# mmorel-35/trivy

Measured on AMD Instinct MI355X. Metric: GB/s secret-scanned (builtin rules) at 1/2/4/8 MI355X; findings diff = 0, higher is better.
Workload: dtype u8

## Files before the change

trivy_amd/csrc/capi.cpp:

```cpp
#include "../../include/trivy_secret.h"
#include "../../include/trivy_secret_test.h"

#include <algorithm>
#include <atomic>
#include <chrono>
#include <memory>
#include <cstdio>
#include <cstdlib>
#include <cstring>
#include <deque>
#include <condition_variable>
#include <mutex>
#include <thread>

#include <malloc.h>
#include <pthread.h>

#include "engine.h"
#include "gosort.h"
#include "guard.h"
#include "inflate_dev.h"
#include "feed.h"
#include "tar.h"
#include "tarscan.h"
// ... 939 lines not shown
  in.paths = paths;
  in.path_lens = path_lens;
  in.binary = binary;
  std::unique_ptr<tsg_result> r(new tsg_result());
  r->rs = rs->rs;
  RawScan raw;
  const std::function<void()> before_confirm = [&] { if (release) release(user); };
  if (!eng->model_scan_device(in, chunk, &r->files, &r->stats, &err, &raw, &before_confirm))
    return fail(TSG_ERR_INTERNAL, err);
  r->raw_segs = std::move(raw.segs);
  *out = r.release();
  return TSG_OK;
  TSG_API_CATCH
}

int tsg_result_raw_segments(const tsg_result* r, size_t* n) {
  TSG_API_TRY
  if (!r || !n) return fail(TSG_ERR_INVALID, "NULL argument");
  *n = r->raw_segs.size();
  return TSG_OK;
  TSG_API_CATCH
}

int tsg_result_raw_segment(const tsg_result* r, size_t k, tsg_raw_segment* rec) {
  TSG_API_TRY
  if (!r || !rec) return fail(TSG_ERR_INVALID, "NULL argument");
  if (k >= r->raw_segs.size()) return fail(TSG_ERR_INVALID, "no such segment");
  const RawSegment& s = r->raw_segs[k];
  rec->f0 = s.f0; rec->nfiles = s.nfiles; rec->lead = s.lead; rec->chunk_bytes = s.chunk;
  rec->b0 = s.b0; rec->bytes = s.bytes; rec->lead_bytes = s.lead_bytes; rec->hits = s.hits;
  rec->lead_flags = s.lead_flags; rec->lead_emitted = s.lead_emitted;
  rec->chunk_newlines = s.nl.data(); rec->nchunks = s.nl.size();
  rec->lead_cand_rules = s.lead_rules.data(); rec->lead_cand_starts = s.lead_starts.data();
  rec->nlead_cands = s.lead_rules.size();
  return TSG_OK;
  TSG_API_CATCH
}

int tsg_test_inject_segment_failures(tsg_engine* e, uint32_t n) {
  TSG_API_TRY
  if (!e) return fail(TSG_ERR_INVALID, "engine is NULL");
  e->eng->inject_segment_failures(n);
  return TSG_OK;
  TSG_API_CATCH
}

int tsg_test_wire_pack(const uint8_t* src, size_t n, int path, uint8_t* packed, size_t packed_cap, uint32_t* table,
                       size_t* packed_len, int* path_used, uint8_t* back) {
  TSG_API_TRY
  if ((!src && n) || !table || !packed_len || (!packed && packed_cap)) return fail(TSG_ERR_INVALID, "NULL argument");
  if (path < 0 || path > 2 || n > kWireMaxStrip) return fail(TSG_ERR_INVALID, "path or length out of range");
  std::vector<uint8_t> buf(wire_bound(n));
  std::vector<uint32_t> tab(wire_blocks(n) + 1);
  const size_t pl = wire_pack(src, n, buf.data(), tab.data(), path);
  *packed_len = pl;
  if (path_used) *path_used = path != kWireScalar && wire_have_avx2() ? kWireAvx2 : kWireScalar;
  if (pl > packed_cap) return fail(TSG_ERR_INVALID, "packed_cap is too small");
  if (pl) memcpy(packed, buf.data(), pl);
  memcpy(table, tab.data(), wire_blocks(n) * sizeof(uint32_t));
  if (back) {
    std::vector<uint8_t> exact(buf.begin(), buf.begin() + pl);
    wire_unpack(exact.data(), tab.data(), n, back);
  }
  return TSG_OK;
  TSG_API_CATCH
}

int tsg_test_wire_unpack_device(const uint8_t* packed, size_t packed_len, const uint32_t* table, size_t n,
                                uint8_t* out) {
  TSG_API_TRY
  if (n && (!packed || !table || !out)) return fail(TSG_ERR_INVALID, "NULL argument");
  const char* msg = "";
  if (!wire_unpack_device_probe(packed, packed_len, table, n, out, &msg)) return fail(TSG_ERR_INTERNAL, msg);
  return TSG_OK;
  TSG_API_CATCH
}

static int test_wire_pack2(const uint8_t* src, size_t n, int path, bool split, uint8_t* packed, size_t packed_cap,
                           uint32_t* table, uint8_t* alpha, size_t* packed_len, int* path_used, uint64_t* counts,
                           uint8_t* back) {
  TSG_API_TRY
  if ((!src && n) || !table || !alpha || !packed_len || (!packed && packed_cap)) return fail(TSG_ERR_INVALID, "NULL argument");
  if (path < 0 || path > 3 || n > kWireMaxStrip) return fail(TSG_ERR_INVALID, "path or length out of range");
  std::vector<uint8_t> buf(wire2_bound(n));
  std::vector<uint32_t> tab(wire_blocks(n) + 1);
  std::vector<uint8_t> al(wire2_alpha_bytes(n) + 1);
  Wire2Stats st;
  const size_t pl = wire_pack2(src, n, buf.data(), tab.data(), al.data(), path, &st, split);
  *packed_len = pl;
  if (path_used) *path_used = wire2_path(path);
  if (counts) { counts[0] = st.blocks6; counts[1] = st.blocks7; counts[2] = st.blocks_raw; counts[3] = st.escaped; }
  if (counts && split) counts[4] = st.blocks_split;
  if (pl > packed_cap) return fail(TSG_ERR_INVALID, "packed_cap is too small");
  if (pl) memcpy(packed, buf.data(), pl);
  memcpy(table, tab.data(), wire_blocks(n) * sizeof(uint32_t));
  memcpy(alpha, al.data(), wire2_alpha_bytes(n));
  if (back) {
    std::vector<uint8_t> exact(buf.begin(), buf.begin() + pl);
    wire_unpack2(exact.data(), tab.data(), al.data(), n, back);
  }
  return TSG_OK;
  TSG_API_CATCH
}

int tsg_test_wire_pack2(const uint8_t* src, size_t n, int path, uint8_t* packed, size_t packed_cap, uint32_t* table,
                        uint8_t* alpha, size_t* packed_len, int* path_used, uint64_t* counts, uint8_t* back) {
  return test_wire_pack2(src, n, path, false, packed, packed_cap, table, alpha, packed_len, path_used, counts, back);
}

int tsg_test_wire_pack3(const uint8_t* src, size_t n, int path, uint8_t* packed, size_t packed_cap, uint32_t* table,
                        uint8_t* alpha, size_t* packed_len, int* path_used, int* vbmi2, uint64_t* counts, uint8_t* back) {
  if (vbmi2) *vbmi2 = wire_have_vbmi2() ? 1 : 0;
  return test_wire_pack2(src, n, path, true, packed, packed_cap, table, alpha, packed_len, path_used, counts, back);
}

int tsg_test_wire_unpack2_device(const uint8_t* packed, size_t packed_len, const uint32_t* table, const uint8_t* alpha,
                                 size_t n, uint8_t* out) {
  TSG_API_TRY
  if (n && (!packed || !table || !alpha || !out)) return fail(TSG_ERR_INVALID, "NULL argument");
  const char* msg = "";
  if (!wire_unpack2_device_probe(packed, packed_len, table, alpha, n, out, &msg)) return fail(TSG_ERR_INTERNAL, msg);
  return TSG_OK;
  TSG_API_CATCH
}

int tsg_test_wire_unpack3_device(const uint8_t* packed, size_t packed_len, const uint32_t* table, const uint8_t* alpha,
                                 size_t n, uint8_t* out) {
  return tsg_test_wire_unpack2_device(packed, packed_len, table, alpha, n, out);
}

static std::string cstr(const char* p) { return p ? std::string(p) : std::string(); }

int tsg_result_from_json(const char* json, size_t len, tsg_result** out) {
  TSG_API_TRY
  if (!json || !out) return fail(TSG_ERR_INVALID, "NULL argument");
  JValue doc;
  std::string err;
  if (!json_parse(std::string(json, len), &doc, &err) || doc.kind != JValue::Arr) return fail(TSG_ERR_INVALID, "json: " + err);
  auto* r = new tsg_result();
  r->own_rules = std::make_shared<std::deque<Rule>>();
  auto sget = [](const JValue* o, const char* k) { const JValue* v = o ? o->get(k) : nullptr; return v ? v->as_string() : std::string(); };
  auto iget = [](const JValue* o, const char* k) { const JValue* v = o ? o->get(k) : nullptr; return v && v->kind == JValue::Num ? static_cast<int>(v->num) : 0; };
  auto bget = [](const JValue* o, const char* k) { const JValue* v = o ? o->get(k) : nullptr; return v && v->kind == JValue::Bool && v->b; };
  auto put = [](SecretBuilder* s, const std::string& v) { return s->put(v.data(), v.size()); };
  for (const auto& js : doc.arr) {
    SecretBuilder s;
    s.file_path = sget(&js, "FilePath");
    const JValue* fs = js.get("Findings");
    if (fs && fs->kind == JValue::Arr) {
      for (const auto& jf : fs->arr) {
        Rule rule;
        rule.id = sget(&jf, "RuleID");
        rule.category = sget(&jf, "Category");
        rule.title = sget(&jf, "Title");
        rule.severity = sget(&jf, "Severity");
        r->own_rules->push_back(rule);
        FindingRec f;
        f.rule = &r->own_rules->back();
        f.start_line = iget(&jf, "StartLine");
        f.end_line = iget(&jf, "EndLine");
        f.match = put(&s, sget(&jf, "Match"));
        f.line_begin = static_cast<uint32_t>(s.lines.size());
        const JValue* code = jf.get("Code");
        const JValue* lines = code ? code->get("Lines") : nullptr;
        if (lines && lines->kind == JValue::Arr) {
          for (const auto& jl : lines->arr) {
            LineRec ln;
            ln.number = iget(&jl, "Number");
            ln.content = put(&s, sget(&jl, "Content"));
            ln.is_cause = bget(&jl, "IsCause");
            ln.first_cause = bget(&jl, "FirstCause");
            ln.last_cause = bget(&jl, "LastCause");
// ... 984 lines not shown
```

trivy_amd/csrc/wirepack.cpp:

```cpp
#include "wirepack.h"

#include <algorithm>
#include <cstring>
#include <memory>

#if defined(__x86_64__)
#include <immintrin.h>
#endif

namespace tsg {

namespace {

constexpr uint64_t kHigh = 0x8080808080808080ull;

inline uint64_t squeeze(uint64_t x) {
  x = (x & 0x007F007F007F007Full) | ((x & 0x7F007F007F007F00ull) >> 1);
  x = (x & 0x00003FFF00003FFFull) | ((x & 0x3FFF00003FFF0000ull) >> 2);
  return (x & 0x000000000FFFFFFFull) | ((x & 0x0FFFFFFF00000000ull) >> 4);
}

inline uint64_t spread(uint64_t v) {
  uint64_t x = (v & 0x000000000FFFFFFFull) | ((v << 4) & 0x0FFFFFFF00000000ull);
  x = (x & 0x00003FFF00003FFFull) | ((x << 2) & 0x3FFF00003FFF0000ull);
  return (x & 0x007F007F007F007Full) | ((x << 1) & 0x7F007F007F007F00ull);
}

inline uint64_t pack_groups_scalar(const uint8_t* src, size_t n, size_t g0, uint8_t* dst) {
  uint64_t acc = 0;
  const size_t ng = n / 8;
  for (size_t g = g0; g < ng; ++g) {
    uint64_t x;
    std::memcpy(&x, src + 8 * g, 8);
    acc |= x;
    x = squeeze(x & ~kHigh);
    std::memcpy(dst + 7 * g, &x, 8);
  }
  if (n % 8) {
    uint64_t x = 0;
    std::memcpy(&x, src + 8 * ng, n % 8);
    acc |= x;
    x = squeeze(x & ~kHigh);
    std::memcpy(dst + 7 * ng, &x, 8);
  }
  return acc;
}

uint64_t pack_block_scalar(const uint8_t* src, size_t n, uint8_t* dst) { return pack_groups_scalar(src, n, 0, dst); }

#if defined(__x86_64__)
__attribute__((target("avx2"))) uint64_t pack_block_avx2(const uint8_t* src, size_t n, uint8_t* dst) {
  const __m256i m1 = _mm256_set1_epi64x(0x007F007F007F007Fll), m1h = _mm256_set1_epi64x(0x7F007F007F007F00ll);
  const __m256i m2 = _mm256_set1_epi64x(0x00003FFF00003FFFll), m2h = _mm256_set1_epi64x(0x3FFF00003FFF0000ll);
  const __m256i m3 = _mm256_set1_epi64x(0x000000000FFFFFFFll), m3h = _mm256_set1_epi64x(0x0FFFFFFF00000000ll);
  const __m256i shuf = _mm256_setr_epi8(0, 1, 2, 3, 4, 5, 6, 8, 9, 10, 11, 12, 13, 14, -1, -1,
                                        0, 1, 2, 3, 4, 5, 6, 8, 9, 10, 11, 12, 13, 14, -1, -1);
  __m256i acc = _mm256_setzero_si256();
  const size_t nv = n / 32;
  for (size_t i = 0; i < nv; ++i) {
    __m256i x = _mm256_loadu_si256(reinterpret_cast<const __m256i*>(src + 32 * i));
    acc = _mm256_or_si256(acc, x);
    x = _mm256_or_si256(_mm256_and_si256(x, m1), _mm256_srli_epi64(_mm256_and_si256(x, m1h), 1));
    x = _mm256_or_si256(_mm256_and_si256(x, m2), _mm256_srli_epi64(_mm256_and_si256(x, m2h), 2));
    x = _mm256_or_si256(_mm256_and_si256(x, m3), _mm256_srli_epi64(_mm256_and_si256(x, m3h), 4));
    x = _mm256_shuffle_epi8(x, shuf);
    _mm_storeu_si128(reinterpret_cast<__m128i*>(dst + 28 * i), _mm256_castsi256_si128(x));
    _mm_storeu_si128(reinterpret_cast<__m128i*>(dst + 28 * i + 14), _mm256_extracti128_si256(x, 1));
  }
  const __m128i a = _mm_or_si128(_mm256_castsi256_si128(acc), _mm256_extracti128_si256(acc, 1));
  uint64_t r = static_cast<uint64_t>(_mm_cvtsi128_si64(a)) | static_cast<uint64_t>(_mm_extract_epi64(a, 1));
  return r | pack_groups_scalar(src, n, nv * 4, dst);
}
#endif

}

bool wire_have_avx2() {
#if defined(__x86_64__)
  static const bool have = __builtin_cpu_supports("avx2");
  return have;
#else
  return false;
#endif
}

size_t wire_pack(const uint8_t* src, size_t n, uint8_t* dst, uint32_t* table, int path) {
  uint64_t (*pack_block)(const uint8_t*, size_t, uint8_t*) = pack_block_scalar;
#if defined(__x86_64__)
  if (path != kWireScalar && wire_have_avx2()) pack_block = pack_block_avx2;
#endif
  size_t o = 0;
  const size_t nb = wire_blocks(n);
  for (size_t b = 0; b < nb; ++b) {
    const uint8_t* s = src + b * kWireBlock;
    const size_t len = n - b * kWireBlock < kWireBlock ? n - b * kWireBlock : kWireBlock;
    if (pack_block(s, len, dst + o) & kHigh) {
      std::memcpy(dst + o, s, len);
      table[b] = static_cast<uint32_t>(o) | kWireRawBit;
      o += len;
    } else {
      table[b] = static_cast<uint32_t>(o);
      o += wire_packed_len(len);
    }
  }
  return o;
}

namespace {

void unpack7_block(const uint8_t* s, size_t len, uint8_t* d) {
  for (size_t g = 0; 8 * g < len; ++g) {
    uint64_t v = 0;
    std::memcpy(&v, s + 7 * g, 7);
    const uint64_t x = spread(v);
    std::memcpy(d + 8 * g, &x, len - 8 * g < 8 ? len - 8 * g : 8);
  }
}

}

void wire_unpack(const uint8_t* packed, const uint32_t* table, size_t n, uint8_t* dst) {
  const size_t nb = wire_blocks(n);
  for (size_t b = 0; b < nb; ++b) {
    const size_t len = n - b * kWireBlock < kWireBlock ? n - b * kWireBlock : kWireBlock;
    const uint8_t* s = packed + (table[b] & ~kWireRawBit);
    uint8_t* d = dst + b * kWireBlock;
    if (table[b] & kWireRawBit) {
      std::memcpy(d, s, len);
      continue;
    }
    unpack7_block(s, len, d);
  }
}


namespace {

constexpr uint32_t kAbort = ~0u;

struct Alphabet {
  uint8_t code[256];
  alignas(64) uint8_t inv[128];
};

void choose_alphabet(const uint8_t* p, size_t len, uint8_t* vals, Alphabet* a) {
  uint32_t key[128];
  for (uint32_t v = 0; v < 128; ++v) key[v] = 127 - v;
  for (size_t i = 0; i < len; i += kWire2Sample)
    if (p[i] < 0x80) key[p[i]] += 256;
  std::partial_sort(key, key + kWire2Escape, key + 128, [](uint32_t x, uint32_t y) { return x > y; });
  std::memset(a->code, kWire2Escape, sizeof a->code);
  std::memset(a->inv, 0, sizeof a->inv);
  for (uint32_t c = 0; c < kWire2Escape; ++c) {
    const uint8_t v = static_cast<uint8_t>(127 - (key[c] & 0xFF));
    vals[c] = v;
    a->code[v] = static_cast<uint8_t>(c);
    a->inv[v] = static_cast<uint8_t>(kWire2Escape - c);
  }
  vals[kWire2Escape] = 0;
}

inline uint32_t pack6_groups_scalar(const uint8_t* src, size_t len, size_t g0, const Alphabet& a, uint8_t* dst,
                                    uint8_t* esc, uint32_t nesc, uint32_t limit, uint32_t* acc) {
  const size_t ng = (len + 3) / 4;
  for (size_t g = g0; g < ng; ++g) {
    uint32_t v = 0;
    const size_t k = len - 4 * g < 4 ? len - 4 * g : 4;
    for (size_t j = 0; j < k; ++j) {
      const uint8_t x = src[4 * g + j];
      const uint32_t c = a.code[x];
      *acc |= x;
      v |= c << (6 * j);
      if (c == kWire2Escape) esc[nesc++] = x;
    }
    dst[3 * g] = static_cast<uint8_t>(v);
    dst[3 * g + 1] = static_cast<uint8_t>(v >> 8);
    dst[3 * g + 2] = static_cast<uint8_t>(v >> 16);
    if (nesc >= limit) return kAbort;
  }
  return nesc;
}

uint32_t pack6_scalar(const uint8_t* src, size_t len, const Alphabet& a, uint8_t* dst, uint8_t* esc, uint32_t limit,
                      uint32_t* acc) {
  return pack6_groups_scalar(src, len, 0, a, dst, esc, 0, limit, acc);
}

#if defined(__x86_64__)
__attribute__((target("avx2"))) uint32_t pack6_avx2(const uint8_t* src, size_t len, const Alphabet& a, uint8_t* dst,
                                                     uint8_t* esc, uint32_t limit, uint32_t* acc) {
  __m256i T[8], X[8];
  for (int k = 0; k < 8; ++k) {
    T[k] = _mm256_broadcastsi128_si256(_mm_load_si128(reinterpret_cast<const __m128i*>(a.inv + 16 * k)));
    X[k] = _mm256_set1_epi8(static_cast<char>(16 * k));
  }
  const __m256i k70 = _mm256_set1_epi8(0x70), k63 = _mm256_set1_epi8(63);
  const __m256i mul1 = _mm256_set1_epi16(0x4001), mul2 = _mm256_set1_epi32(0x10000001);
  const __m256i shuf = _mm256_setr_epi8(0, 1, 2, 4, 5, 6, 8, 9, 10, 12, 13, 14, -1, -1, -1, -1,
                                        0, 1, 2, 4, 5, 6, 8, 9, 10, 12, 13, 14, -1, -1, -1, -1);
  __m256i vacc = _mm256_setzero_si256();
  uint32_t nesc = 0;
  const size_t nv = len / 32;
  for (size_t i = 0; i < nv; ++i) {
    const __m256i x = _mm256_loadu_si256(reinterpret_cast<const __m256i*>(src + 32 * i));
    vacc = _mm256_or_si256(vacc, x);
    __m256i r = _mm256_shuffle_epi8(T[0], _mm256_adds_epu8(x, k70));
    for (int k = 1; k < 8; ++k)
      r = _mm256_or_si256(r, _mm256_shuffle_epi8(T[k], _mm256_adds_epu8(_mm256_xor_si256(x, X[k]), k70)));
    const __m256i c = _mm256_sub_epi8(k63, r);
    uint32_t m = static_cast<uint32_t>(_mm256_movemask_epi8(_mm256_cmpeq_epi8(c, k63)));
    __m256i p = _mm256_madd_epi16(_mm256_maddubs_epi16(c, mul1), mul2);
    p = _mm256_shuffle_epi8(p, shuf);
    _mm_storeu_si128(reinterpret_cast<__m128i*>(dst + 24 * i), _mm256_castsi256_si128(p));
    _mm_storeu_si128(reinterpret_cast<__m128i*>(dst + 24 * i + 12), _mm256_extracti128_si256(p, 1));
    if (m) {
      for (; m; m &= m - 1) esc[nesc++] = src[32 * i + static_cast<unsigned>(__builtin_ctz(m))];
      if (nesc >= limit) return kAbort;
    }
  }
  const __m128i v = _mm_or_si128(_mm256_castsi256_si128(vacc), _mm256_extracti128_si256(vacc, 1));
  const uint64_t r = static_cast<uint64_t>(_mm_cvtsi128_si64(v)) | static_cast<uint64_t>(_mm_extract_epi64(v, 1));
  *acc |= (r & kHigh) ? 0x80u : 0u;
  return pack6_groups_scalar(src, len, nv * 8, a, dst, esc, nesc, limit, acc);
}

__attribute__((target("avx512f,avx512bw,avx512vl,avx512vbmi"))) uint32_t pack6_vbmi(const uint8_t* src, size_t len,
                                                                                     const Alphabet& a, uint8_t* dst,
                                                                                     uint8_t* esc, uint32_t limit,
                                                                                     uint32_t* acc) {
  const __m512i t0 = _mm512_load_si512(a.inv), t1 = _mm512_load_si512(a.inv + 64);
  const __m512i k63 = _mm512_set1_epi8(63);
  const __m512i mul1 = _mm512_set1_epi16(0x4001), mul2 = _mm512_set1_epi32(0x10000001);
  alignas(64) uint8_t idx[64];
  for (int j = 0; j < 64; ++j) idx[j] = static_cast<uint8_t>(j < 48 ? j / 3 * 4 + j % 3 : 0);
  const __m512i gather = _mm512_load_si512(idx);
  __mmask64 high = 0;
  uint32_t nesc = 0;
  const size_t nv = len / 64;
  for (size_t i = 0; i < nv; ++i) {
// ... 48 lines not shown
#endif


struct Split {
  alignas(64) uint8_t mask[kWireBlock / 8 + 64];
  alignas(64) uint8_t nib[kWireBlock + 128];
  alignas(64) uint8_t five[kWireBlock + 128];
  alignas(64) uint8_t esc[kWireBlock + 128];
  uint32_t h = 0, e = 0;
  uint32_t e6 = 0;
  bool high = false;
};

inline void split_finish(Split* s, size_t len, uint32_t h, uint32_t e, uint32_t e6, bool high) {
  std::memset(s->nib + h, 0, 64);
  std::memset(s->five + (len - h), 0, 64);
  s->h = h; s->e = e; s->e6 = e6; s->high = high;
}

inline void split_scan_codes(const uint8_t* src, const uint8_t* code, size_t i0, size_t len, Split* s, uint32_t h,
                             uint32_t e, uint32_t e6, uint32_t acc) {
  uint32_t w = static_cast<uint32_t>(i0) - h;
  for (size_t i = i0; i < len; ++i) {
    const uint8_t x = src[i], c = code[i];
    acc |= x;
    if (i % 8 == 0) s->mask[i / 8] = 0;
    if (c < kWire2Hot) {
      s->mask[i / 8] |= static_cast<uint8_t>(1u << (i % 8));
      s->nib[h++] = c;
    } else if (c < kWire2Warm) {
      s->five[w++] = static_cast<uint8_t>(c - kWire2Hot);
    } else {
      s->five[w++] = kWire2Escape5;
      s->esc[e++] = x;
      e6 += c == kWire2Escape;
    }
  }
  split_finish(s, len, h, e, e6, (acc & 0x80) != 0);
}

void split_scan_scalar(const uint8_t* src, size_t len, const Alphabet& a, Split* s) {
  uint8_t code[kWireBlock];
  for (size_t i = 0; i < len; ++i) code[i] = a.code[src[i]];
  split_scan_codes(src, code, 0, len, s, 0, 0, 0, 0);
}

void split_emit_scalar(const Split& s, size_t len, uint8_t* d) {
  const size_t M = (len + 7) / 8, N = (s.h + 1) / 2, nf = len - s.h, F = (5 * nf + 7) / 8;
  std::memcpy(d, s.mask, M);
  d += M;
  for (size_t j = 0; j < N; ++j) d[j] = static_cast<uint8_t>(s.nib[2 * j] | s.nib[2 * j + 1] << 4);
  d += N;
  for (size_t g = 0; 5 * g < F; ++g) {
    uint64_t v = 0;
    for (int j = 0; j < 8; ++j) v |= static_cast<uint64_t>(s.five[8 * g + j]) << (5 * j);
    for (size_t j = 0; j < 5 && 5 * g + j < F; ++j) d[5 * g + j] = static_cast<uint8_t>(v >> (8 * j));
  }
  d += F;
  std::memcpy(d, s.esc, s.e);
  std::memset(d + s.e, 0, wire2_split_bytes(len, s.h, s.e) - (M + N + F + s.e));
}

#if defined(__x86_64__)
__attribute__((target("avx2"))) void split_scan_avx2(const uint8_t* src, size_t len, const Alphabet& a, Split* s) {
  __m256i T[8], X[8];
  for (int k = 0; k < 8; ++k) {
    T[k] = _mm256_broadcastsi128_si256(_mm_load_si128(reinterpret_cast<const __m128i*>(a.inv + 16 * k)));
    X[k] = _mm256_set1_epi8(static_cast<char>(16 * k));
  }
  const __m256i k70 = _mm256_set1_epi8(0x70), k63 = _mm256_set1_epi8(63);
  alignas(32) uint8_t code[kWireBlock];
  const size_t nv = len / 32;
  for (size_t i = 0; i < nv; ++i) {
    const __m256i x = _mm256_loadu_si256(reinterpret_cast<const __m256i*>(src + 32 * i));
    __m256i r = _mm256_shuffle_epi8(T[0], _mm256_adds_epu8(x, k70));
    for (int k = 1; k < 8; ++k)
      r = _mm256_or_si256(r, _mm256_shuffle_epi8(T[k], _mm256_adds_epu8(_mm256_xor_si256(x, X[k]), k70)));
    _mm256_store_si256(reinterpret_cast<__m256i*>(code + 32 * i), _mm256_sub_epi8(k63, r));
  }
  for (size_t i = 32 * nv; i < len; ++i) code[i] = a.code[src[i]];
  split_scan_codes(src, code, 0, len, s, 0, 0, 0, 0);
}

__attribute__((target("avx512f,avx512bw,avx512vl,avx512vbmi,avx512vbmi2"))) void split_scan_vbmi2(
    const uint8_t* src, size_t len, const Alphabet& a, Split* s) {
  const __m512i t0 = _mm512_load_si512(a.inv), t1 = _mm512_load_si512(a.inv + 64);
  const __m512i k63 = _mm512_set1_epi8(63), khot = _mm512_set1_epi8(static_cast<char>(kWire2Hot));
  const __m512i kwarm = _mm512_set1_epi8(static_cast<char>(kWire2Warm)), k31 = _mm512_set1_epi8(kWire2Escape5);
  uint32_t h = 0, w = 0, e = 0, e6 = 0;
  __mmask64 high = 0;
  for (size_t i = 0; i < len; i += 64) {
    const __mmask64 valid = len - i >= 64 ? ~0ull : (1ull << (len - i)) - 1;
    const __m512i x = _mm512_maskz_loadu_epi8(valid, src + i);
    const __mmask64 hi = _mm512_movepi8_mask(x);
    high |= hi;
    const __m512i r = _mm512_permutex2var_epi8(t0, x, t1);
    const __m512i c = _mm512_mask_mov_epi8(_mm512_sub_epi8(k63, r), hi, k63);
    const __mmask64 hot = _mm512_cmplt_epu8_mask(c, khot) & valid, rest = ~hot & valid;
    const uint64_t hot_bits = hot;
    std::memcpy(s->mask + i / 8, &hot_bits, 8);
    _mm512_storeu_si512(s->nib + h, _mm512_maskz_compress_epi8(hot, c));
    h += static_cast<uint32_t>(__builtin_popcountll(hot));
    const __m512i f = _mm512_min_epu8(_mm512_sub_epi8(c, khot), k31);
    _mm512_storeu_si512(s->five + w, _mm512_maskz_compress_epi8(rest, f));
    w += static_cast<uint32_t>(__builtin_popcountll(rest));
    const __mmask64 out = _mm512_cmpge_epu8_mask(c, kwarm) & valid;
    if (out) {
      _mm512_storeu_si512(s->esc + e, _mm512_maskz_compress_epi8(out, x));
      e += static_cast<uint32_t>(__builtin_popcountll(out));
      e6 += static_cast<uint32_t>(__builtin_popcountll(_mm512_cmpeq_epi8_mask(c, k63) & valid));
    }
  }
  split_finish(s, len, h, e, e6, high != 0);
}

__attribute__((target("avx512f,avx512bw,avx512vl,avx512vbmi"))) void split_emit_vbmi(const Split& s, size_t len,
                                                                                     uint8_t* d) {
  const size_t M = (len + 7) / 8, N = (s.h + 1) / 2, nf = len - s.h, F = (5 * nf + 7) / 8;
  std::memcpy(d, s.mask, M);
  d += M;
  const __m512i two = _mm512_set1_epi16(0x1001);
  for (size_t j = 0; j < s.h; j += 64) {
    const __m512i v = _mm512_load_si512(s.nib + j);
    _mm256_storeu_si256(reinterpret_cast<__m256i*>(d + j / 2), _mm512_cvtepi16_epi8(_mm512_maddubs_epi16(v, two)));
  }
  d += N;
  alignas(64) uint8_t idx[64];
  for (int j = 0; j < 64; ++j) idx[j] = static_cast<uint8_t>(j < 40 ? j / 5 * 8 + j % 5 : 5);
  const __m512i gather = _mm512_load_si512(idx);
  const __m512i mul1 = _mm512_set1_epi16(0x2001), mul2 = _mm512_set1_epi32(0x04000001);
  const __m512i lo20 = _mm512_set1_epi64(0xFFFFF), hi20 = _mm512_set1_epi64(0xFFFFF00000ll);
  for (size_t j = 0; j < nf; j += 64) {
    const __m512i v = _mm512_load_si512(s.five + j);
    const __m512i q = _mm512_madd_epi16(_mm512_maddubs_epi16(v, mul1), mul2);
    const __m512i p = _mm512_or_si512(_mm512_and_si512(q, lo20), _mm512_and_si512(_mm512_srli_epi64(q, 12), hi20));
    _mm512_storeu_si512(d + j / 8 * 5, _mm512_permutexvar_epi8(gather, p));
  }
  d += F;
  std::memcpy(d, s.esc, s.e);
  std::memset(d + s.e, 0, wire2_split_bytes(len, s.h, s.e) - (M + N + F + s.e));
}
#endif

}

bool wire_have_vbmi() {
#if defined(__x86_64__)
  static const bool have = __builtin_cpu_supports("avx512f") && __builtin_cpu_supports("avx512bw") &&
                           __builtin_cpu_supports("avx512vl") && __builtin_cpu_supports("avx512vbmi");
  return have;
#else
  return false;
#endif
}

bool wire_have_vbmi2() {
#if defined(__x86_64__)
  static const bool have = wire_have_vbmi() && __builtin_cpu_supports("avx512vbmi2");
  return have;
#else
  return false;
#endif
}

int wire2_path(int path) {
  if (path == kWireScalar) return kWireScalar;
  if (path != kWireAvx2 && wire_have_vbmi()) return kWireVbmi;
  return wire_have_avx2() ? kWireAvx2 : kWireScalar;
}

size_t wire_pack2(const uint8_t* src, size_t n, uint8_t* dst, uint32_t* table, uint8_t* alpha, int path,
                  Wire2Stats* stats, bool split) {
  uint32_t (*pack6)(const uint8_t*, size_t, const Alphabet&, uint8_t*, uint8_t*, uint32_t, uint32_t*) = pack6_scalar;
  uint64_t (*pack7)(const uint8_t*, size_t, uint8_t*) = pack_block_scalar;
  void (*split_scan)(const uint8_t*, size_t, const Alphabet&, Split*) = split_scan_scalar;
  void (*split_emit)(const Split&, size_t, uint8_t*) = split_emit_scalar;
#if defined(__x86_64__)
  const int used = wire2_path(path);
  if (used != kWireScalar) pack7 = pack_block_avx2;
  if (used == kWireAvx2) pack6 = pack6_avx2;
  if (used == kWireVbmi) pack6 = wire_have_vbmi2() ? pack6_vbmi2 : pack6_vbmi;
  if (used != kWireScalar) { split_scan = split_scan_avx2; }
  if (used == kWireVbmi) split_emit = split_emit_vbmi;
  if (used == kWireVbmi && wire_have_vbmi2()) split_scan = split_scan_vbmi2;
#endif
  if (n) std::memset(alpha, 0, wire2_alpha_bytes(n));
  Wire2Stats st;
  Alphabet a;
  uint8_t esc[kWireBlock + 64];
  std::unique_ptr<Split> sp(split ? new Split : nullptr);
  size_t o = 0;
  const size_t nb = wire_blocks(n);
  for (size_t b = 0; b < nb; ++b) {
    const size_t at = b * kWireBlock;
    if (at % kWire2Region == 0)
      choose_alphabet(src + at, n - at < kWire2Region ? n - at : kWire2Region, alpha + at / kWire2Region * kWire2Alpha, &a);
    const uint8_t* s = src + at;
    const size_t len = n - at < kWireBlock ? n - at : kWireBlock;
    const size_t cb = wire2_code_bytes(len);
    const uint32_t limit = len > cb ? static_cast<uint32_t>(len - cb) : 0;
    uint32_t acc = 0;
    bool no6 = false;
    if (split) {
      split_scan(s, len, a, sp.get());
      const size_t size7 = sp->high ? len : wire_packed_len(len), size6 = cb + ((sp->e6 + 15) & ~size_t(15));
      const size_t sizes = wire2_split_bytes(len, sp->h, sp->e);
      if (sizes < len && sizes < size7 && sizes < size6) {
        split_emit(*sp, len, dst + o);
        table[b] = static_cast<uint32_t>(o) | kWireRawBit | kWire6Bit;
        o += sizes;
        ++st.blocks_split;
        st.escaped += sp->e;
        continue;
      }
      no6 = !(size6 < len && size6 < size7);
    }
    const uint32_t nesc = limit && !no6 ? pack6(s, len, a, dst + o, esc, limit, &acc) : kAbort;
    if (nesc != kAbort) {
      const size_t size6 = cb + ((nesc + 15) & ~size_t(15));
      const bool ascii = !(acc & 0x80);
      if (size6 < len && !(ascii && wire_packed_len(len) <= size6)) {
        const size_t codes = (len + 3) / 4 * 3;
        std::memset(dst + o + codes, 0, cb - codes);
        std::memcpy(dst + o + cb, esc, nesc);
        std::memset(dst + o + cb + nesc, 0, size6 - cb - nesc);
        table[b] = static_cast<uint32_t>(o) | kWire6Bit;
        o += size6;
        ++st.blocks6;
        st.escaped += nesc;
        continue;
      }
    }
    if (wire_packed_len(len) < len && !(pack7(s, len, dst + o) & kHigh)) {
      table[b] = static_cast<uint32_t>(o);
      o += wire_packed_len(len);
      ++st.blocks7;
    } else {
      std::memcpy(dst + o, s, len);
      table[b] = static_cast<uint32_t>(o) | kWireRawBit;
      o += len;
      ++st.blocks_raw;
    }
  }
  if (stats) *stats = st;
  return o;
}

void wire_unpack2(const uint8_t* packed, const uint32_t* table, const uint8_t* alpha, size_t n, uint8_t* dst) {
  const size_t nb = wire_blocks(n);
  for (size_t b = 0; b < nb; ++b) {
    const size_t at = b * kWireBlock;
    const size_t len = n - at < kWireBlock ? n - at : kWireBlock;
    const uint8_t* s = packed + (table[b] & ~(kWireRawBit | kWire6Bit));
    uint8_t* d = dst + at;
    if ((table[b] & kWireRawBit) && (table[b] & kWire6Bit)) {
      const uint8_t* al = alpha + at / kWire2Region * kWire2Alpha;
      size_t h = 0;
      for (size_t i = 0; i < len; ++i) h += s[i / 8] >> (i % 8) & 1;
      const uint8_t* nib = s + (len + 7) / 8;
      const uint8_t* five = nib + (h + 1) / 2;
      const uint8_t* e = five + (5 * (len - h) + 7) / 8;
      size_t jn = 0, jf = 0;
      for (size_t i = 0; i < len; ++i) {
        if (s[i / 8] >> (i % 8) & 1) {
          d[i] = al[nib[jn / 2] >> (4 * (jn % 2)) & 15];
          ++jn;
        } else {
          const size_t bit = 5 * jf++;
          const uint32_t lo = five[bit >> 3], hi = (bit & 7) > 3 ? five[(bit >> 3) + 1] : 0;
          const uint32_t c = ((lo | hi << 8) >> (bit & 7)) & 31;
          d[i] = c == kWire2Escape5 ? *e++ : al[kWire2Hot + c];
        }
      }
    } else if (table[b] & kWireRawBit) {
      std::memcpy(d, s, len);
    } else if (table[b] & kWire6Bit) {
      const uint8_t* al = alpha + at / kWire2Region * kWire2Alpha;
      const uint8_t* e = s + wire2_code_bytes(len);
      for (size_t i = 0; i < len; ++i) {
        const size_t bit = 6 * i;
        const uint32_t lo = s[bit >> 3], hi = (bit & 7) > 2 ? s[(bit >> 3) + 1] : 0;
        const uint32_t c = ((lo | hi << 8) >> (bit & 7)) & 63;
        d[i] = c == kWire2Escape ? *e++ : al[c];
      }
    } else {
      unpack7_block(s, len, d);
    }
  }
}

}
```

trivy_amd/csrc/wirepack.h:

```cpp
#pragma once
#include <cstddef>
#include <cstdint>

namespace tsg {

constexpr uint32_t kWireBlock = 4096;
constexpr uint32_t kWireBlockPacked = kWireBlock / 8 * 7;
constexpr uint32_t kWireRawBit = 1u << 31;
constexpr uint64_t kWireMaxStrip = 1ull << 30;
constexpr size_t kWireSlack = 64;

enum WirePath { kWireAuto = 0, kWireScalar = 1, kWireAvx2 = 2, kWireVbmi = 3 };

inline size_t wire_blocks(size_t n) { return (n + kWireBlock - 1) / kWireBlock; }
inline size_t wire_packed_len(size_t block_bytes) { return (block_bytes + 7) / 8 * 7; }
inline size_t wire_bound(size_t n) { return n + 8 + kWireSlack; }
inline size_t wire_table_bytes(size_t n) { return (wire_blocks(n) * sizeof(uint32_t) + 255) & ~size_t(255); }

bool wire_have_avx2();
size_t wire_pack(const uint8_t* src, size_t n, uint8_t* dst, uint32_t* table, int path);
void wire_unpack(const uint8_t* packed, const uint32_t* table, size_t n, uint8_t* dst);

bool wire_unpack_device_probe(const uint8_t* packed, size_t packed_len, const uint32_t* table, size_t n, uint8_t* out,
                              const char** err);


constexpr uint32_t kWire6Bit = 1u << 30;
constexpr uint32_t kWire2Region = 65536;
constexpr uint32_t kWire2Sample = 64;
constexpr uint32_t kWire2Alpha = 64;
constexpr uint32_t kWire2Escape = 63;

struct Wire2Stats {
  uint64_t blocks6 = 0, blocks7 = 0, blocks_raw = 0;
  uint64_t escaped = 0;
  uint64_t blocks_split = 0;
};

inline size_t wire2_regions(size_t n) { return (n + kWire2Region - 1) / kWire2Region; }
inline size_t wire2_alpha_bytes(size_t n) { return (wire2_regions(n) * kWire2Alpha + 255) & ~size_t(255); }
inline size_t wire2_code_bytes(size_t block_bytes) { return ((block_bytes + 3) / 4 * 3 + 15) & ~size_t(15); }
inline size_t wire2_bound(size_t n) { return n + 16 + kWireSlack; }
constexpr uint32_t kWire2Hot = 16;
constexpr uint32_t kWire2Warm = 47;
constexpr uint32_t kWire2Escape5 = 31;
inline size_t wire2_split_bytes(size_t len, size_t h, size_t e) {
  return ((len + 7) / 8 + (h + 1) / 2 + (5 * (len - h) + 7) / 8 + e + 15) & ~size_t(15);
}

bool wire_have_vbmi();
bool wire_have_vbmi2();
int wire2_path(int path);
size_t wire_pack2(const uint8_t* src, size_t n, uint8_t* dst, uint32_t* table, uint8_t* alpha, int path,
                  Wire2Stats* stats, bool split = false);
void wire_unpack2(const uint8_t* packed, const uint32_t* table, const uint8_t* alpha, size_t n, uint8_t* dst);
bool wire_unpack2_device_probe(const uint8_t* packed, size_t packed_len, const uint32_t* table, const uint8_t* alpha,
                               size_t n, uint8_t* out, const char** err);

}
```

Before: 74.28.

## Vectorize wire2 split scan/emit with AVX-512 and speed up alphabet ranking

Replaces the split-mode host packing path with AVX-512 VBMI2 routines: a scan that stores codes, nibble and 5-bit values plus escapes into a new VScan buffer, then vectorized nibble/five-bit packing and a 6-bit code emitter. It also adds an optional merge variant that packs on the fly, a histogram-plus-SIMD ranking in place of partial_sort for alphabet choice, and software prefetch of upcoming source and destination. The intent is to cut host-side CPU cost of wire compression before device upload. It adds complexity and scratch memory, and ordering ties in the rank path could differ from partial_sort.

```diff
diff --git a/trivy_amd/csrc/capi.cpp b/trivy_amd/csrc/capi.cpp
--- a/trivy_amd/csrc/capi.cpp
+++ b/trivy_amd/csrc/capi.cpp
@@ -1045,12 +1045,15 @@
   TSG_API_TRY
   if ((!src && n) || !table || !alpha || !packed_len || (!packed && packed_cap)) return fail(TSG_ERR_INVALID, "NULL argument");
   if (path < 0 || path > 3 || n > kWireMaxStrip) return fail(TSG_ERR_INVALID, "path or length out of range");
-  std::vector<uint8_t> buf(wire2_bound(n));
+  constexpr size_t kGuard = 64;
+  std::vector<uint8_t> buf(wire2_bound(n) + kGuard, 0xA5);
   std::vector<uint32_t> tab(wire_blocks(n) + 1);
   std::vector<uint8_t> al(wire2_alpha_bytes(n) + 1);
   Wire2Stats st;
   const size_t pl = wire_pack2(src, n, buf.data(), tab.data(), al.data(), path, &st, split);
   *packed_len = pl;
+  for (size_t i = 0; i < kGuard; ++i)
+    if (buf[wire2_bound(n) + i] != 0xA5) return fail(TSG_ERR_INTERNAL, "wire_pack2 wrote past wire2_bound(n)");
   if (path_used) *path_used = wire2_path(path);
   if (counts) { counts[0] = st.blocks6; counts[1] = st.blocks7; counts[2] = st.blocks_raw; counts[3] = st.escaped; }
   if (counts && split) counts[4] = st.blocks_split;
diff --git a/trivy_amd/csrc/wirepack.cpp b/trivy_amd/csrc/wirepack.cpp
--- a/trivy_amd/csrc/wirepack.cpp
+++ b/trivy_amd/csrc/wirepack.cpp
@@ -2,6 +2,7 @@
 
 #include <algorithm>
 #include <cstring>
+#include <functional>
 #include <memory>
 
 #if defined(__x86_64__)
@@ -137,24 +138,71 @@
 namespace {
 
 constexpr uint32_t kAbort = ~0u;
+#ifndef TSG_WIRE_PREFETCH
+#define TSG_WIRE_PREFETCH 1
+#endif
+constexpr bool kWirePrefetch = TSG_WIRE_PREFETCH != 0;
 
 struct Alphabet {
   uint8_t code[256];
   alignas(64) uint8_t inv[128];
 };
 
-void choose_alphabet(const uint8_t* p, size_t len, uint8_t* vals, Alphabet* a) {
-  uint32_t key[128];
-  for (uint32_t v = 0; v < 128; ++v) key[v] = 127 - v;
-  for (size_t i = 0; i < len; i += kWire2Sample)
-    if (p[i] < 0x80) key[p[i]] += 256;
-  std::partial_sort(key, key + kWire2Escape, key + 128, [](uint32_t x, uint32_t y) { return x > y; });
-  std::memset(a->code, kWire2Escape, sizeof a->code);
+#if defined(__x86_64__)
+__attribute__((target("avx512f,avx512bw,avx512vl"))) void rank_keys_avx512(const uint32_t* key, uint8_t* rank) {
+  __m512i K[8], R[8];
+  for (int j = 0; j < 8; ++j) {
+    K[j] = _mm512_load_si512(key + 16 * j);
+    R[j] = _mm512_setzero_si512();
+  }
+  const __m512i one = _mm512_set1_epi32(1);
+  for (int v = 0; v < 128; ++v) {
+    const __m512i b = _mm512_set1_epi32(static_cast<int>(key[v]));
+    for (int j = 0; j < 8; ++j) R[j] = _mm512_mask_add_epi32(R[j], _mm512_cmpgt_epu32_mask(b, K[j]), R[j], one);
+  }
+  for (int j = 0; j < 8; ++j) _mm_store_si128(reinterpret_cast<__m128i*>(rank + 16 * j), _mm512_cvtepi32_epi8(R[j]));
+}
+#endif
+
+void choose_alphabet(const uint8_t* p, size_t len, uint8_t* vals, Alphabet* a, bool want_code) {
+  uint16_t hist[4][128];
+  std::memset(hist, 0, sizeof hist);
+  const size_t ns = (len + kWire2Sample - 1) / kWire2Sample;
+  size_t s = 0;
+  for (; s + 4 <= ns; s += 4) {
+    const uint8_t b0 = p[kWire2Sample * s], b1 = p[kWire2Sample * (s + 1)];
+    const uint8_t b2 = p[kWire2Sample * (s + 2)], b3 = p[kWire2Sample * (s + 3)];
+    hist[0][b0 & 127] += static_cast<uint16_t>((b0 >> 7) ^ 1);
+    hist[1][b1 & 127] += static_cast<uint16_t>((b1 >> 7) ^ 1);
+    hist[2][b2 & 127] += static_cast<uint16_t>((b2 >> 7) ^ 1);
+    hist[3][b3 & 127] += static_cast<uint16_t>((b3 >> 7) ^ 1);
+  }
+  for (; s < ns; ++s) hist[0][p[kWire2Sample * s] & 127] += static_cast<uint16_t>((p[kWire2Sample * s] >> 7) ^ 1);
+  alignas(64) uint32_t key[128];
+  for (uint32_t v = 0; v < 128; ++v)
+    key[v] = static_cast<uint32_t>(hist[0][v] + hist[1][v] + hist[2][v] + hist[3][v]) << 8 | (127 - v);
+  if (want_code) std::memset(a->code, kWire2Escape, sizeof a->code);
   std::memset(a->inv, 0, sizeof a->inv);
+#if defined(__x86_64__)
+  if (wire_have_vbmi()) {
+    alignas(64) uint8_t rank[128], order[128];
+    rank_keys_avx512(key, rank);
+    for (uint32_t v = 0; v < 128; ++v) {
+      const uint32_t c = rank[v];
+      order[c] = static_cast<uint8_t>(v);
+      a->inv[v] = static_cast<uint8_t>(c < kWire2Escape ? kWire2Escape - c : 0);
+      if (want_code) a->code[v] = static_cast<uint8_t>(c < kWire2Escape ? c : kWire2Escape);
+    }
+    std::memcpy(vals, order, kWire2Escape);
+    vals[kWire2Escape] = 0;
+    return;
+  }
+#endif
+  std::partial_sort(key, key + kWire2Escape, key + 128, std::greater<uint32_t>());
   for (uint32_t c = 0; c < kWire2Escape; ++c) {
     const uint8_t v = static_cast<uint8_t>(127 - (key[c] & 0xFF));
     vals[c] = v;
-    a->code[v] = static_cast<uint8_t>(c);
+    if (want_code) a->code[v] = static_cast<uint8_t>(c);
     a->inv[v] = static_cast<uint8_t>(kWire2Escape - c);
   }
   vals[kWire2Escape] = 0;
@@ -369,36 +417,177 @@
   split_scan_codes(src, code, 0, len, s, 0, 0, 0, 0);
 }
 
-__attribute__((target("avx512f,avx512bw,avx512vl,avx512vbmi,avx512vbmi2"))) void split_scan_vbmi2(
-    const uint8_t* src, size_t len, const Alphabet& a, Split* s) {
+struct VScan {
+  alignas(64) uint8_t esc[kWireBlock + 64];
+  alignas(64) uint8_t code[kWireBlock];
+  alignas(64) uint8_t nib[kWireBlock + 128];
+  alignas(64) uint8_t val5[kWireBlock + 128];
+  alignas(64) uint8_t five[kWireBlock / 8 * 5 + 64];
+  uint32_t h = 0, e = 0, e6 = 0;
+  bool high = false;
+};
+
+struct VTables {
+  alignas(64) uint8_t rotate[64][64];
+  alignas(64) uint64_t waiting[128];
+  alignas(64) uint8_t gather4[64], gather5[64], gather6[64];
+  constexpr VTables() : rotate(), waiting(), gather4(), gather5(), gather6() {
+    for (int w = 0; w < 64; ++w) {
+      for (int j = 0; j < 64; ++j) rotate[w][j] = static_cast<uint8_t>((j - w) & 63);
+      waiting[w] = (1ull << w) - 1;
+    }
+    for (int j = 0; j < 64; ++j) {
+      gather4[j] = static_cast<uint8_t>(j < 32 ? 2 * j : 1);
+      gather5[j] = static_cast<uint8_t>(j < 40 ? j / 5 * 8 + j % 5 : 7);
+      gather6[j] = static_cast<uint8_t>(j < 48 ? j / 3 * 4 + j % 3 : 3);
+    }
+  }
+};
+constexpr VTables kV;
+
+#define TSG_VBMI2 __attribute__((target("avx512f,avx512bw,avx512vl,avx512vbmi,avx512vbmi2,popcnt")))
+
+TSG_VBMI2 inline __m256i pack_nibbles(__m512i v, __m512i gather) {
+  return _mm512_castsi512_si256(_mm512_permutexvar_epi8(gather, _mm512_maddubs_epi16(v, _mm512_set1_epi16(0x1001))));
+}
+
+TSG_VBMI2 inline __m512i pack_fives(__m512i v, __m512i gather) {
+  const __m512i q = _mm512_madd_epi16(_mm512_maddubs_epi16(v, _mm512_set1_epi16(0x2001)), _mm512_set1_epi32(0x04000001));
+  const __m512i p = _mm512_ternarylogic_epi64(q, _mm512_srli_epi64(q, 12), _mm512_set1_epi64(0xFFFFF00000ll), 0xD8);
+  return _mm512_permutexvar_epi8(gather, p);
+}
+
+TSG_VBMI2 void split_merge_vbmi2(const uint8_t* src, size_t len, const Alphabet& a, uint8_t* d, VScan* s) {
+  const __m512i t0 = _mm512_load_si512(a.inv), t1 = _mm512_load_si512(a.inv + 64);
+  const __m512i k63 = _mm512_set1_epi8(63), khot = _mm512_set1_epi8(static_cast<char>(kWire2Hot));
+  const __m512i kwarm = _mm512_set1_epi8(static_cast<char>(kWire2Warm)), k31 = _mm512_set1_epi8(kWire2Escape5);
+  const __m512i gather4 = _mm512_load_si512(kV.gather4), gather5 = _mm512_load_si512(kV.gather5);
+  uint8_t* dn = d + (len + 7) / 8;
+  uint8_t* df = s->five;
+  __m512i pn = _mm512_setzero_si512(), pf = _mm512_setzero_si512();
+  uint32_t wn = 0, wf = 0;
+  uint32_t h = 0, e = 0, e6 = 0;
+  __mmask64 high = 0;
+  for (size_t i = 0; i < len; i += 64) {
+    const size_t rem = len - i;
+    const __mmask64 valid = rem >= 64 ? ~0ull : (1ull << rem) - 1;
+    const __m512i x = _mm512_maskz_loadu_epi8(valid, src + i);
+    const __mmask64 hi = _mm512_movepi8_mask(x);
+    high |= hi;
+    const __m512i r = _mm512_permutex2var_epi8(t0, x, t1);
+    const __m512i c = _mm512_maskz_mov_epi8(valid, _mm512_mask_mov_epi8(_mm512_sub_epi8(k63, r), hi, k63));
+    _mm512_store_si512(s->code + i, c);
+    const __mmask64 hot = _mm512_cmplt_epu8_mask(c, khot) & valid, rest = ~hot & valid;
+    const uint64_t hot_bits = hot;
+    if (rem >= 64) std::memcpy(d + i / 8, &hot_bits, 8);
+    else std::memcpy(d + i / 8, &hot_bits, (rem + 7) / 8);
+    {
+      const uint32_t k = static_cast<uint32_t>(__builtin_popcountll(hot));
+      const __mmask64 waiting = static_cast<__mmask64>(kV.waiting[wn]);
+      const __m512i rot = _mm512_permutexvar_epi8(_mm512_load_si512(kV.rotate[wn]), _mm512_maskz_compress_epi8(hot, c));
+      _mm256_storeu_si256(reinterpret_cast<__m256i*>(dn), pack_nibbles(_mm512_mask_mov_epi8(rot, waiting, pn), gather4));
+      const uint64_t full = (wn + k) >> 6;
+      pn = _mm512_mask_mov_epi8(rot, static_cast<__mmask64>(kV.waiting[wn + 64 * full]), pn);
+      dn += full << 5;
+      wn = (wn + k) & 63;
+      h += k;
+    }
+    {
+      const uint32_t k = static_cast<uint32_t>(__builtin_popcountll(rest));
+      const __mmask64 waiting = static_cast<__mmask64>(kV.waiting[wf]);
+      const __m512i f = _mm512_min_epu8(_mm512_sub_epi8(c, khot), k31);
+      const __m512i rot = _mm512_permutexvar_epi8(_mm512_load_si512(kV.rotate[wf]), _mm512_maskz_compress_epi8(rest, f));
+      _mm512_storeu_si512(df, pack_fives(_mm512_mask_mov_epi8(rot, waiting, pf), gather5));
+      const uint64_t full = (wf + k) >> 6;
+      pf = _mm512_mask_mov_epi8(rot, static_cast<__mmask64>(kV.waiting[wf + 64 * full]), pf);
+      df += full * 40;
+      wf = (wf + k) & 63;
+    }
+    const __mmask64 out = _mm512_cmpge_epu8_mask(c, kwarm) & valid;
+    _mm512_storeu_si512(s->esc + e, _mm512_maskz_compress_epi8(out, x));
+    e += static_cast<uint32_t>(__builtin_popcountll(out));
+    e6 += static_cast<uint32_t>(__builtin_popcountll(_mm512_cmpeq_epi8_mask(c, k63) & valid));
+  }
+  _mm256_storeu_si256(reinterpret_cast<__m256i*>(dn), pack_nibbles(_mm512_maskz_mov_epi8((1ull << wn) - 1, pn), gather4));
+  _mm512_storeu_si512(df, pack_fives(_mm512_maskz_mov_epi8((1ull << wf) - 1, pf), gather5));
+  s->h = h; s->e = e; s->e6 = e6; s->high = high != 0;
+}
+
+TSG_VBMI2 void split_scan_vbmi2(const uint8_t* src, size_t len, const Alphabet& a, uint8_t* d, VScan* s) {
   const __m512i t0 = _mm512_load_si512(a.inv), t1 = _mm512_load_si512(a.inv + 64);
   const __m512i k63 = _mm512_set1_epi8(63), khot = _mm512_set1_epi8(static_cast<char>(kWire2Hot));
   const __m512i kwarm = _mm512_set1_epi8(static_cast<char>(kWire2Warm)), k31 = _mm512_set1_epi8(kWire2Escape5);
   uint32_t h = 0, w = 0, e = 0, e6 = 0;
   __mmask64 high = 0;
   for (size_t i = 0; i < len; i += 64) {
-    const __mmask64 valid = len - i >= 64 ? ~0ull : (1ull << (len - i)) - 1;
+    const size_t rem = len - i;
+    const __mmask64 valid = rem >= 64 ? ~0ull : (1ull << rem) - 1;
     const __m512i x = _mm512_maskz_loadu_epi8(valid, src + i);
     const __mmask64 hi = _mm512_movepi8_mask(x);
     high |= hi;
     const __m512i r = _mm512_permutex2var_epi8(t0, x, t1);
-    const __m512i c = _mm512_mask_mov_epi8(_mm512_sub_epi8(k63, r), hi, k63);
+    const __m512i c = _mm512_maskz_mov_epi8(valid, _mm512_mask_mov_epi8(_mm512_sub_epi8(k63, r), hi, k63));
+    _mm512_store_si512(s->code + i, c);
     const __mmask64 hot = _mm512_cmplt_epu8_mask(c, khot) & valid, rest = ~hot & valid;
     const uint64_t hot_bits = hot;
-    std::memcpy(s->mask + i / 8, &hot_bits, 8);
+    if (rem >= 64) std::memcpy(d + i / 8, &hot_bits, 8);
+    else std::memcpy(d + i / 8, &hot_bits, (rem + 7) / 8);
     _mm512_storeu_si512(s->nib + h, _mm512_maskz_compress_epi8(hot, c));
     h += static_cast<uint32_t>(__builtin_popcountll(hot));
     const __m512i f = _mm512_min_epu8(_mm512_sub_epi8(c, khot), k31);
-    _mm512_storeu_si512(s->five + w, _mm512_maskz_compress_epi8(rest, f));
+    _mm512_storeu_si512(s->val5 + w, _mm512_maskz_compress_epi8(rest, f));
     w += static_cast<uint32_t>(__builtin_popcountll(rest));
     const __mmask64 out = _mm512_cmpge_epu8_mask(c, kwarm) & valid;
-    if (out) {
-      _mm512_storeu_si512(s->esc + e, _mm512_maskz_compress_epi8(out, x));
-      e += static_cast<uint32_t>(__builtin_popcountll(out));
-      e6 += static_cast<uint32_t>(__builtin_popcountll(_mm512_cmpeq_epi8_mask(c, k63) & valid));
-    }
-  }
-  split_finish(s, len, h, e, e6, high != 0);
+    _mm512_storeu_si512(s->esc + e, _mm512_maskz_compress_epi8(out, x));
+    e += static_cast<uint32_t>(__builtin_popcountll(out));
+    e6 += static_cast<uint32_t>(__builtin_popcountll(_mm512_cmpeq_epi8_mask(c, k63) & valid));
+  }
+  _mm512_storeu_si512(s->nib + h, _mm512_setzero_si512());
+  _mm512_storeu_si512(s->val5 + w, _mm512_setzero_si512());
+  s->h = h; s->e = e; s->e6 = e6; s->high = high != 0;
+}
+
+TSG_VBMI2 void split_emit_vbmi2(const VScan& s, size_t len, uint8_t* d) {
+  const size_t M = (len + 7) / 8, N = (s.h + 1) / 2, nf = len - s.h, F = (5 * nf + 7) / 8;
+  const __m512i gather4 = _mm512_load_si512(kV.gather4), gather5 = _mm512_load_si512(kV.gather5);
+  d += M;
+  for (size_t j = 0; j < s.h; j += 64)
+    _mm256_storeu_si256(reinterpret_cast<__m256i*>(d + j / 2), pack_nibbles(_mm512_load_si512(s.nib + j), gather4));
+  d += N;
+  for (size_t j = 0; j < nf; j += 64) _mm512_storeu_si512(d + j / 8 * 5, pack_fives(_mm512_load_si512(s.val5 + j), gather5));
+  d += F;
+  std::memcpy(d, s.esc, s.e);
+  std::memset(d + s.e, 0, wire2_split_bytes(len, s.h, s.e) - (M + N + F + s.e));
+}
+
+inline void split_merge_finish(const VScan& s, size_t len, uint8_t* d) {
+  const size_t M = (len + 7) / 8, N = (s.h + 1) / 2, F = (5 * (len - s.h) + 7) / 8;
+  d += M + N;
+  std::memcpy(d, s.five, F);
+  std::memcpy(d + F, s.esc, s.e);
+  std::memset(d + F + s.e, 0, wire2_split_bytes(len, s.h, s.e) - (M + N + F + s.e));
+}
+
+TSG_VBMI2 void emit6_codes_vbmi2(const uint8_t* src, size_t len, const VScan& s, uint8_t* d) {
+  const __m512i mul1 = _mm512_set1_epi16(0x4001), mul2 = _mm512_set1_epi32(0x10000001);
+  const __m512i gather = _mm512_load_si512(kV.gather6), k63 = _mm512_set1_epi8(63);
+  for (size_t i = 0; i < len; i += 64) {
+    const __m512i c = _mm512_load_si512(s.code + i);
+    const __m512i p = _mm512_madd_epi16(_mm512_maddubs_epi16(c, mul1), mul2);
+    _mm512_storeu_si512(d + i / 64 * 48, _mm512_permutexvar_epi8(gather, p));
+  }
+  const size_t codes = (len + 3) / 4 * 3, cb = wire2_code_bytes(len);
+  std::memset(d + codes, 0, cb - codes);
+  uint32_t nesc = 0;
+  for (size_t i = 0; nesc < s.e6; i += 64) {
+    const __mmask64 m = _mm512_cmpeq_epi8_mask(_mm512_load_si512(s.code + i), k63);
+    if (!m) continue;
+    const size_t rem = len - i;
+    const __m512i x = _mm512_maskz_loadu_epi8(rem >= 64 ? ~0ull : (1ull << rem) - 1, src + i);
+    _mm512_storeu_si512(d + cb + nesc, _mm512_maskz_compress_epi8(m, x));
+    nesc += static_cast<uint32_t>(__builtin_popcountll(m));
+  }
+  std::memset(d + cb + nesc, 0, ((nesc + 15) & ~size_t(15)) - nesc);
 }
 
 __attribute__((target("avx512f,avx512bw,avx512vl,avx512vbmi"))) void split_emit_vbmi(const Split& s, size_t len,
@@ -451,6 +640,7 @@
 }
 
 int wire2_path(int path) {
+  if (path == kWireVbmiMerge) path = kWireVbmi;
   if (path == kWireScalar) return kWireScalar;
   if (path != kWireAvx2 && wire_have_vbmi()) return kWireVbmi;
   return wire_have_avx2() ? kWireAvx2 : kWireScalar;
@@ -469,25 +659,60 @@
   if (used == kWireVbmi) pack6 = wire_have_vbmi2() ? pack6_vbmi2 : pack6_vbmi;
   if (used != kWireScalar) { split_scan = split_scan_avx2; }
   if (used == kWireVbmi) split_emit = split_emit_vbmi;
-  if (used == kWireVbmi && wire_have_vbmi2()) split_scan = split_scan_vbmi2;
+  const bool vscan = split && used == kWireVbmi && wire_have_vbmi2();
+  const bool merge = path == kWireVbmiMerge;
+  std::unique_ptr<VScan> op(vscan ? new VScan : nullptr);
+#else
+  const bool vscan = false;
 #endif
   if (n) std::memset(alpha, 0, wire2_alpha_bytes(n));
   Wire2Stats st;
   Alphabet a;
   uint8_t esc[kWireBlock + 64];
-  std::unique_ptr<Split> sp(split ? new Split : nullptr);
+  std::unique_ptr<Split> sp(split && !vscan ? new Split : nullptr);
   size_t o = 0;
   const size_t nb = wire_blocks(n);
   for (size_t b = 0; b < nb; ++b) {
     const size_t at = b * kWireBlock;
     if (at % kWire2Region == 0)
-      choose_alphabet(src + at, n - at < kWire2Region ? n - at : kWire2Region, alpha + at / kWire2Region * kWire2Alpha, &a);
+      choose_alphabet(src + at, n - at < kWire2Region ? n - at : kWire2Region, alpha + at / kWire2Region * kWire2Alpha, &a,
+                      !vscan);
     const uint8_t* s = src + at;
     const size_t len = n - at < kWireBlock ? n - at : kWireBlock;
+    if (kWirePrefetch) {
+      for (size_t k = 0; k < kWireBlock; k += 64) __builtin_prefetch(s + kWire2Region + k, 0, 2);
+      for (size_t k = 0; k < kWireBlock; k += 64) __builtin_prefetch(dst + o + 2 * kWireBlock + k, 1, 3);
+    }
     const size_t cb = wire2_code_bytes(len);
     const uint32_t limit = len > cb ? static_cast<uint32_t>(len - cb) : 0;
     uint32_t acc = 0;
     bool no6 = false;
+#if defined(__x86_64__)
+    if (vscan) {
+      if (merge) split_merge_vbmi2(s, len, a, dst + o, op.get());
+      else split_scan_vbmi2(s, len, a, dst + o, op.get());
+      const size_t size7 = op->high ? len : wire_packed_len(len), size6 = cb + ((op->e6 + 15) & ~size_t(15));
+      const size_t sizes = wire2_split_bytes(len, op->h, op->e);
+      if (sizes < len && sizes < size7 && sizes < size6) {
+        if (merge) split_merge_finish(*op, len, dst + o);
+        else split_emit_vbmi2(*op, len, dst + o);
+        table[b] = static_cast<uint32_t>(o) | kWireRawBit | kWire6Bit;
+        o += sizes;
+        ++st.blocks_split;
+        st.escaped += op->e;
+        continue;
+      }
+      if (size6 < len && size6 < size7) {
+        emit6_codes_vbmi2(s, len, *op, dst + o);
+        table[b] = static_cast<uint32_t>(o) | kWire6Bit;
+        o += size6;
+        ++st.blocks6;
+        st.escaped += op->e6;
+        continue;
+      }
+      no6 = true;
+    } else
+#endif
     if (split) {
       split_scan(s, len, a, sp.get());
       const size_t size7 = sp->high ? len : wire_packed_len(len), size6 = cb + ((sp->e6 + 15) & ~size_t(15));
@@ -531,6 +756,44 @@
   }
   if (stats) *stats = st;
   return o;
+}
+
+uint64_t wire2_probe(const uint8_t* src, size_t n, uint8_t* dst, uint8_t* alpha, int path, int what) {
+  const int used = wire2_path(path);
+  void (*split_scan)(const uint8_t*, size_t, const Alphabet&, Split*) = split_scan_scalar;
+#if defined(__x86_64__)
+  if (used != kWireScalar) split_scan = split_scan_avx2;
+  const bool vscan = used == kWireVbmi && wire_have_vbmi2();
+  const bool merge = path == kWireVbmiMerge;
+  std::unique_ptr<VScan> op(vscan ? new VScan : nullptr);
+#else
+  const bool vscan = false;
+#endif
+  std::unique_ptr<Split> sp(vscan ? nullptr : new Split);
+  Alphabet a;
+  uint64_t sum = 0;
+  size_t o = 0;
+  for (size_t at = 0; at < n; at += kWireBlock) {
+    if (at % kWire2Region == 0) {
+      uint8_t* vals = alpha + at / kWire2Region * kWire2Alpha;
+      choose_alphabet(src + at, n - at < kWire2Region ? n - at : kWire2Region, vals, &a, !vscan);
+      sum += vals[0] + 256u * vals[kWire2Escape - 1];
+    }
+    if (what == kWireProbeAlphabet) continue;
+    const size_t len = n - at < kWireBlock ? n - at : kWireBlock;
+#if defined(__x86_64__)
+    if (vscan) {
+      if (merge) split_merge_vbmi2(src + at, len, a, dst + o, op.get());
+      else split_scan_vbmi2(src + at, len, a, dst + o, op.get());
+      sum += op->h + op->e + op->e6;
+      o += wire2_split_bytes(len, op->h, 0) < len ? wire2_split_bytes(len, op->h, 0) : len;
+      continue;
+    }
+#endif
+    split_scan(src + at, len, a, sp.get());
+    sum += sp->h + sp->e + sp->e6;
+  }
+  return sum;
 }
 
 void wire_unpack2(const uint8_t* packed, const uint32_t* table, const uint8_t* alpha, size_t n, uint8_t* dst) {
diff --git a/trivy_amd/csrc/wirepack.h b/trivy_amd/csrc/wirepack.h
--- a/trivy_amd/csrc/wirepack.h
+++ b/trivy_amd/csrc/wirepack.h
@@ -10,7 +10,8 @@
 constexpr uint64_t kWireMaxStrip = 1ull << 30;
 constexpr size_t kWireSlack = 64;
 
-enum WirePath { kWireAuto = 0, kWireScalar = 1, kWireAvx2 = 2, kWireVbmi = 3 };
+enum WirePath { kWireAuto = 0, kWireScalar = 1, kWireAvx2 = 2, kWireVbmi = 3,
+                kWireVbmiMerge = 4 };
 
 inline size_t wire_blocks(size_t n) { return (n + kWireBlock - 1) / kWireBlock; }
 inline size_t wire_packed_len(size_t block_bytes) { return (block_bytes + 7) / 8 * 7; }
@@ -53,6 +54,8 @@
 int wire2_path(int path);
 size_t wire_pack2(const uint8_t* src, size_t n, uint8_t* dst, uint32_t* table, uint8_t* alpha, int path,
                   Wire2Stats* stats, bool split = false);
+enum WireProbe { kWireProbeAlphabet = 0, kWireProbeScan = 1 };
+uint64_t wire2_probe(const uint8_t* src, size_t n, uint8_t* dst, uint8_t* alpha, int path, int what);
 void wire_unpack2(const uint8_t* packed, const uint32_t* table, const uint8_t* alpha, size_t n, uint8_t* dst);
 bool wire_unpack2_device_probe(const uint8_t* packed, size_t packed_len, const uint32_t* table, const uint8_t* alpha,
                                size_t n, uint8_t* out, const char** err);
```

After: 76.22 (median of 5 runs). 1.03x the previous value.
